# michal-szadkowski/rl-selfplay-mnk

Measured on AMD Instinct MI355X. Metric: env-steps/sec 9x9x5, 65536 parallel envs/GPU, random-policy rollout, higher is better.
Workload: dtype u64

## Files before the change

include/mnk_hip.h:

```cpp
#ifndef MNK_HIP_H
#define MNK_HIP_H

#ifndef __HIPCC_RTC__
#include <stddef.h>
#include <stdint.h>
#endif

#ifdef __cplusplus
extern "C" {
#endif

#define MNK_ABI_VERSION 6

#define MNK_OK 0
#define MNK_EINVAL -1
#define MNK_EGEOM -2
#define MNK_ELAUNCH -3
#define MNK_ECOMM -4

#define MNK_ERR_NONE 0
#define MNK_ERR_ACTION_RANGE 1
#define MNK_ERR_ILLEGAL_MOVE 2
#define MNK_ERR_SYMMETRY 3
#define MNK_ERR_VISITS 4
// ... 252 lines not shown
#define MNK_JIT_REPLAY 1
#define MNK_JIT_ROLLOUT_PAIR 2
int64_t mnk_jit_compile_kernel(int m, int n, int k, int record, int act_bytes, int kind);
const char* mnk_jit_last_error(void);
#define MNK_JIT_API_STEP 0
#define MNK_JIT_API_STEP_DRAW 1
#define MNK_JIT_API_STEP_SUBSET 2
#define MNK_JIT_API_OBSERVE 3
#define MNK_JIT_API_SAMPLE_LEGAL 4
#define MNK_JIT_API_UNPACK_RECORDS 5
#define MNK_JIT_API_GATHER_OBS 6
#define MNK_JIT_API_SP_PRE 7
#define MNK_JIT_API_SP_POST 8
#define MNK_JIT_API_SP_STEP 9
#define MNK_JIT_API_SP_DRAW 10
#define MNK_JIT_API_SP_TACTICAL 19
#define MNK_JIT_API_SP_TACTICAL_DRAW 20
#define MNK_JIT_API_SAMPLE_TACTICAL 23
#define MNK_JIT_API_COUNT 24
int64_t mnk_jit_compile_api(int m, int n, int k, int kind);
int mnk_jit_prepare(int m, int n, int k, int64_t kinds);
int mnk_jit_stats(int64_t* out4);
int mnk_jit_api_ready(int m, int n, int k, int kind);

int mnk_action_log_words(int act_bytes, int T);
int mnk_replay_actions(uint64_t* planes, uint32_t* meta, int64_t N, int m, int n, int k, int T,
                       const void* act_log, int act_bytes, uint64_t* rec_planes, uint32_t* rec_meta,
                       int32_t* err, void* stream);

int mnk_unpack_records(const uint64_t* rec_planes, const uint32_t* rec_meta, int64_t N, int T, int m, int n,
                       void* obs, int obs_dtype, uint8_t* masks, int64_t* actions, float* rewards, uint8_t* dones,
                       void* stream);

int mnk_gather_obs(const uint64_t* planes, int64_t T, int64_t N, int m, int n, const int64_t* idx, int64_t B,
                   void* obs, int obs_dtype, uint8_t* legal_mask, int fix_empty_mask, int32_t* err, void* stream);

int mnk_gae(const float* rewards, const float* values, const uint8_t* dones, const float* last_values,
            int64_t N, int T, float gamma, float gamma_lambda, float* advantages, float* returns,
            void* stream);

int mnk_comm_unique_id(void* id_out_host);
int mnk_comm_init(void** comm_out, const void* id_host, int nranks, int rank);
int mnk_comm_destroy(void* comm);
int mnk_allgather_records(void* comm, const void* send, void* recv, int64_t bytes, void* stream);
int mnk_allgather_records_direct(void* comm, const void* send, void* recv, int64_t bytes, void* stream);
const char* mnk_comm_last_error(void);
int mnk_comm_version(void);

int mnk_probe_record_writes(uint64_t* rec, int64_t N, int T, int rows, void* stream);

int mnk_probe_select_bits(const uint32_t* words, int nw, int64_t count, const int32_t* ranks, int32_t* bits, uint32_t* hot,
                          void* stream);

#ifdef __cplusplus
}
#endif
#endif
```

rl-selfplay-mnk_amd/csrc/mnk_device.h:

```cpp
#pragma once
#ifdef __HIPCC_RTC__
typedef unsigned char uint8_t;
typedef unsigned short uint16_t;
typedef unsigned int uint32_t;
typedef unsigned long long uint64_t;
typedef signed char int8_t;
typedef int int32_t;
typedef long long int64_t;
typedef unsigned long long uintptr_t;
#include "mnk_hip.h"
#else
#include <hip/hip_runtime.h>
#include <stdint.h>

#include "../../include/mnk_hip.h"
#endif

#define MNK_MAX_W 16
#define MNK_MAX_NW 32

struct MnkGeom {
  int m, n, k;
  int C;
  int W;
// ... 123 lines not shown
#pragma unroll
    for (int w = 0; w < NW; ++w) lj[w] = ~0u;
#pragma unroll UK
    for (int j = 0; j < k; ++j) {
      if (j > 0) {
        uint32_t t[NW];
#pragma unroll
        for (int w = 0; w < NW; ++w) t[w] = plane[w];
        bs_shl<NW>(t, j * d);
#pragma unroll
        for (int w = 0; w < NW; ++w) lj[w] &= t[w];
      }
      uint32_t rj[NW];
#pragma unroll
      for (int w = 0; w < NW; ++w) rj[w] = ~0u;
#pragma unroll UK
      for (int i = 1; i < k - j; ++i) {
        uint32_t t[NW];
#pragma unroll
        for (int w = 0; w < NW; ++w) t[w] = plane[w];
        bs_shr<NW>(t, i * d);
#pragma unroll
        for (int w = 0; w < NW; ++w) rj[w] &= t[w];
      }
#pragma unroll
      for (int w = 0; w < NW; ++w) acc[w] |= lj[w] & rj[w];
    }
  }
#pragma unroll
  for (int w = 0; w < NW; ++w) out[w] = acc[w] & empty[w];
}

#define MNK_SELECT_LEVEL(S)                        \
  "v_bfe_u32 %[t], %[x], %[pos], " #S "\n\t"       \
  "v_bcnt_u32_b32 %[t], %[t], %[nr]\n\t"          \
  "v_max_u32 %[nr], %[nr], %[t]\n\t"              \
  "v_ashrrev_i32 %[t], 31, %[t]\n\t"              \
  "v_and_or_b32 %[pos], %[t], " #S ", %[pos]\n\t"
__device__ __forceinline__ uint32_t select_bit32_nr(uint32_t x, uint32_t nr, uint32_t base) {
  uint32_t pos, t;
  asm("v_and_b32 %[t], 0xffff, %[x]\n\t"
      "v_bcnt_u32_b32 %[t], %[t], %[nr]\n\t"
      "v_max_u32 %[nr], %[nr], %[t]\n\t"
      "v_ashrrev_i32 %[t], 31, %[t]\n\t"
      "v_and_or_b32 %[pos], %[t], 16, %[base]\n\t"
      MNK_SELECT_LEVEL(8) MNK_SELECT_LEVEL(4) MNK_SELECT_LEVEL(2)
      "v_bfe_u32 %[t], %[x], %[pos], 1\n\t"
      "v_bitop3_b32 %[t], %[nr], %[t], %[t] bitop3:0x3f\n\t"
      "v_and_or_b32 %[pos], %[t], 1, %[pos]"
      : [pos] "=&v"(pos), [t] "=&v"(t), [nr] "+v"(nr)
      : [x] "v"(x), [base] "v"(base));
  return pos;
}
#undef MNK_SELECT_LEVEL

__device__ __forceinline__ int select_bit32(uint32_t x, int r) { return (int)select_bit32_nr(x, ~(uint32_t)r, 0u); }

template <int NW>
__device__ __forceinline__ int bs_popcount(const uint32_t (&x)[NW]) {
  int c = 0;
#pragma unroll
  for (int w = 0; w < NW; ++w) c += __popc(x[w]);
  return c;
}

template <int NW>
__device__ __forceinline__ int bs_select_hot(const uint32_t (&x)[NW], int r_, uint32_t (&hot)[NW]) {
  const uint32_t nr = ~(uint32_t)r_;
  uint32_t m[NW + 1], word = x[0], base = 0u, rank = nr, pre = 0u;
  m[0] = ~0u;
  m[NW] = 0u;
#pragma unroll
  for (int w = 1; w < NW; ++w) {
    pre += (uint32_t)__popc(x[w - 1]);
    const uint32_t t = pre + nr;
    m[w] = (uint32_t)((int32_t)t >> 31);
    rank = rank > t ? rank : t;
    word = __builtin_amdgcn_bitop3_b32(m[w], x[w], word, 0xca);
    base = __builtin_amdgcn_bitop3_b32(m[w], 32u * w, base, 0xca);
  }
  const uint32_t pos = select_bit32_nr(word, rank, base);
  const uint32_t one = 1u << (pos & 31u);
#pragma unroll
  for (int w = 0; w < NW; ++w) hot[w] = __builtin_amdgcn_bitop3_b32(one, m[w], m[w + 1], 0x40);
  return (int)pos;
}

template <int NW>
__device__ __forceinline__ int bs_select(const uint32_t (&x)[NW], int r) {
  uint32_t hot[NW];
  return bs_select_hot<NW>(x, r, hot);
}

struct Philox4 { uint32_t v[4]; };

__device__ __forceinline__ uint64_t mnk_mul_wide(uint32_t a, uint32_t m) {
  uint64_t product, carry;
  asm("v_mad_u64_u32 %0, %1, %2, %3, 0" : "=v"(product), "=s"(carry) : "v"(a), "s"(m));
  return product;
}
__device__ __forceinline__ uint64_t mnk_mul_wide_vcc(uint32_t a, uint32_t m) {
  uint64_t product;
  asm("v_mad_u64_u32 %0, vcc, %1, %2, 0" : "=v"(product) : "v"(a), "s"(m) : "vcc");
  return product;
}

#define MNK_PHILOX_M0 0xD2511F53u
#define MNK_PHILOX_M1 0xCD9E8D57u

__device__ __forceinline__ uint64_t philox_first_product(uint32_t c0) { return mnk_mul_wide_vcc(c0, MNK_PHILOX_M0); }

__device__ __forceinline__ Philox4 philox4x32_10_from(uint64_t p0_first, uint32_t c1, uint32_t c2, uint32_t c3,
                                                      uint32_t k0, uint32_t k1) {
  uint64_t A[11], B[11];
  uint32_t n0[11], n2[11];
#define MNK_PHILOX_N0(r) \
  n0[r] = __builtin_amdgcn_bitop3_b32((uint32_t)(B[r] >> 32), (r) == 1 ? c1 : (uint32_t)B[(r) - 1], k0 + ((r) - 1) * 0x9E3779B9u, 0x96)
#define MNK_PHILOX_N2(r) \
  n2[r] = __builtin_amdgcn_bitop3_b32((uint32_t)(A[r] >> 32), (r) == 1 ? c3 : (uint32_t)A[(r) - 1], k1 + ((r) - 1) * 0xBB67AE85u, 0x96)
  A[1] = p0_first;
  B[1] = mnk_mul_wide(c2, MNK_PHILOX_M1);
  MNK_PHILOX_N2(1);
#pragma unroll
  for (int r = 2; r <= 10; r += 2) {
    B[r] = mnk_mul_wide(n2[r - 1], MNK_PHILOX_M1);
    MNK_PHILOX_N0(r - 1);
    A[r] = mnk_mul_wide_vcc(n0[r - 1], MNK_PHILOX_M0);
    MNK_PHILOX_N0(r);
    if (r < 10) {
      A[r + 1] = mnk_mul_wide_vcc(n0[r], MNK_PHILOX_M0);
      MNK_PHILOX_N2(r);
      B[r + 1] = mnk_mul_wide(n2[r], MNK_PHILOX_M1);
      MNK_PHILOX_N2(r + 1);
    }
  }
  MNK_PHILOX_N2(10);
#undef MNK_PHILOX_N0
#undef MNK_PHILOX_N2
  Philox4 o;
  o.v[0] = n0[10]; o.v[1] = (uint32_t)B[10]; o.v[2] = n2[10]; o.v[3] = (uint32_t)A[10];
  return o;
}

__device__ __forceinline__ Philox4 philox4x32_10(uint32_t c0, uint32_t c1, uint32_t c2, uint32_t c3,
                                                 uint32_t k0, uint32_t k1) {
#pragma unroll
  for (int r = 0; r < 10; ++r) {
    const uint64_t p0 = mnk_mul_wide(c0, MNK_PHILOX_M0), p1 = mnk_mul_wide(c2, MNK_PHILOX_M1);
    const uint32_t n0 = __builtin_amdgcn_bitop3_b32((uint32_t)(p1 >> 32), c1, k0, 0x96);
    const uint32_t n2 = __builtin_amdgcn_bitop3_b32((uint32_t)(p0 >> 32), c3, k1, 0x96);
    c0 = n0; c1 = (uint32_t)p1; c2 = n2; c3 = (uint32_t)p0;
    k0 += 0x9E3779B9u; k1 += 0xBB67AE85u;
  }
  Philox4 o;
  o.v[0] = c0; o.v[1] = c1; o.v[2] = c2; o.v[3] = c3;
  return o;
}

__device__ __forceinline__ Philox4 mnk_rng_block(uint64_t seed, uint64_t env, uint64_t q, uint32_t stream) {
  return philox4x32_10((uint32_t)env, (uint32_t)(env >> 32), (uint32_t)q,
                       stream | ((uint32_t)((q >> 32) & 0xFFFFFFu) << 8),
                       (uint32_t)seed, (uint32_t)(seed >> 32));
}

__device__ __forceinline__ Philox4 mnk_rng_block_from(uint64_t seed, uint64_t env_p0, uint64_t env, uint64_t q,
                                                      uint32_t stream) {
  return philox4x32_10_from(env_p0, (uint32_t)(env >> 32), (uint32_t)q,
                            stream | ((uint32_t)((q >> 32) & 0xFFFFFFu) << 8),
                            (uint32_t)seed, (uint32_t)(seed >> 32));
}

__device__ __forceinline__ uint32_t philox_word(const Philox4& b, uint32_t i) {
  uint32_t lo = (i & 1u) ? b.v[1] : b.v[0];
  uint32_t hi = (i & 1u) ? b.v[3] : b.v[2];
  return (i & 2u) ? hi : lo;
}

__device__ __forceinline__ uint32_t mnk_rand_u32(uint64_t seed, uint64_t env, uint64_t step, uint32_t stream) {
  Philox4 b = mnk_rng_block(seed, env, step >> 2, stream);
  return philox_word(b, (uint32_t)(step & 3));
}

template <int NW>
struct MnkEnv {
  uint32_t p[2][NW];
  uint32_t meta;
};

template <int NW, bool EXACT = false>
__device__ __forceinline__ void plane_load(uint32_t (&x)[NW], const uint64_t* plane, int64_t N, int W, int64_t i) {
#pragma unroll
  for (int q = 0; q < (NW + 1) / 2; ++q) {
    const uint64_t v = (EXACT || q < W) ? plane[(int64_t)q * N + i] : 0ull;
    x[2 * q] = (uint32_t)v;
    if (2 * q + 1 < NW) x[2 * q + 1] = (uint32_t)(v >> 32);
  }
}

template <int NW, bool EXACT = false>
__device__ __forceinline__ void plane_store(const uint32_t (&x)[NW], uint64_t* plane, int64_t N, int W, int64_t i) {
#pragma unroll
  for (int q = 0; q < (NW + 1) / 2; ++q) {
    const uint64_t hi = (2 * q + 1 < NW) ? (uint64_t)x[2 * q + 1] : 0ull;
    if (EXACT || q < W) plane[(int64_t)q * N + i] = (uint64_t)x[2 * q] | (hi << 32);
  }
}

template <int NW, bool EXACT = false>
__device__ __forceinline__ void rec_store(const uint32_t (&p0)[NW], const uint32_t (&p1)[NW], uint64_t* rows, int64_t N,
                                          int nw, int64_t i) {
#pragma unroll
  for (int w = 0; w < NW; ++w)
    if (EXACT || w < nw) rows[(int64_t)w * N + i] = (uint64_t)p0[w] | ((uint64_t)p1[w] << 32);
}

template <int NW, bool EXACT = false>
__device__ __forceinline__ void rec_load(uint32_t (&p0)[NW], uint32_t (&p1)[NW], const uint64_t* rows, int64_t N, int nw,
                                         int64_t i) {
#pragma unroll
  for (int w = 0; w < NW; ++w) {
    const uint64_t v = (EXACT || w < nw) ? rows[(int64_t)w * N + i] : 0ull;
    p0[w] = (uint32_t)v;
// ... 131 lines not shown
```

rl-selfplay-mnk_amd/csrc/mnk_kernels.hip:

```cpp
#include "mnk_host.h"
#include "mnk_api_kernels.h"
#include "mnk_selfplay_host.h"

__global__ void k_reset_idx(uint64_t* planes, uint32_t* meta, int64_t N, int W, const int64_t* idx, int64_t R,
                            int32_t* err) {
  const int64_t j = (int64_t)blockIdx.x * blockDim.x + threadIdx.x;
  if (j >= R) return;
  int64_t i = idx[j];
  if (i < 0) i += N;
  if (i < 0 || i >= N) { mnk_report(err, MNK_ERR_ACTION_RANGE, idx[j]); return; }
  for (int w = 0; w < 2 * W; ++w) planes[(int64_t)w * N + i] = 0ull;
  meta[i] = 0u;
}

__global__ void k_reset_mask(uint64_t* planes, uint32_t* meta, int64_t N, int W, const uint8_t* mask) {
  const int64_t i = (int64_t)blockIdx.x * blockDim.x + threadIdx.x;
  if (i >= N || !mask[i]) return;
  for (int w = 0; w < 2 * W; ++w) planes[(int64_t)w * N + i] = 0ull;
  meta[i] = 0u;
}

__global__ void k_pack_boards(MnkGeom g, const float* boards, uint64_t* planes, int64_t N) {
  const int64_t i = (int64_t)blockIdx.x * blockDim.x + threadIdx.x;
  if (i >= N) return;
// ... 71 lines not shown
    next_v = v;
  }
}

__global__ void __launch_bounds__(64) k_probe_record_writes(uint64_t* rec, int64_t N, int T, int rows, uint64_t seed) {
  const int64_t i = (int64_t)blockIdx.x * 64 + threadIdx.x;
  if (i >= N) return;
  uint64_t v = seed + (uint64_t)i;
  uint64_t* p = rec + i;
  for (int t = 0; t < T; ++t)
    for (int r = 0; r < rows; ++r) {
      __builtin_nontemporal_store(v + (uint64_t)r, p);
      p += N;
    }
}

template <int NW>
__global__ void __launch_bounds__(64) k_probe_select_bits(const uint32_t* words, int64_t count, const int32_t* ranks,
                                                          int32_t* bits, uint32_t* hot) {
  const int64_t i = (int64_t)blockIdx.x * 64 + threadIdx.x;
  if (i >= count) return;
  uint32_t x[NW], h[NW];
#pragma unroll
  for (int w = 0; w < NW; ++w) x[w] = words[i * NW + w];
  bits[i] = bs_select_hot<NW>(x, ranks[i], h);
#pragma unroll
  for (int w = 0; w < NW; ++w) hot[i * NW + w] = h[w];
}

extern "C" {

int mnk_probe_record_writes(uint64_t* rec, int64_t N, int T, int rows, void* stream) {
  if (!rec || N < 0 || T < 0 || rows < 1) return MNK_EINVAL;
  if (N == 0 || T == 0) return MNK_OK;
  hipLaunchKernelGGL(k_probe_record_writes, dim3((unsigned)((N + 63) / 64)), dim3(64), 0, (hipStream_t)stream, rec, N, T,
                     rows, 0x9E3779B97F4A7C15ull);
  return mnk_launch_status("probe_record_writes");
}

int mnk_probe_select_bits(const uint32_t* words, int nw, int64_t count, const int32_t* ranks, int32_t* bits, uint32_t* hot,
                          void* stream) {
  if (!words || !ranks || !bits || !hot || count < 0 || (nw != 1 && nw != 3 && nw != 12)) return MNK_EINVAL;
  if (count == 0) return MNK_OK;
  const dim3 grid((unsigned)((count + 63) / 64));
  if (nw == 1)
    hipLaunchKernelGGL(k_probe_select_bits<1>, grid, dim3(64), 0, (hipStream_t)stream, words, count, ranks, bits, hot);
  else if (nw == 3)
    hipLaunchKernelGGL(k_probe_select_bits<3>, grid, dim3(64), 0, (hipStream_t)stream, words, count, ranks, bits, hot);
  else
    hipLaunchKernelGGL(k_probe_select_bits<12>, grid, dim3(64), 0, (hipStream_t)stream, words, count, ranks, bits, hot);
  return mnk_launch_status("probe_select_bits");
}

int mnk_abi_version(void) { return MNK_ABI_VERSION; }

int mnk_reload_config(void) {
  mnk_config(true);
  return MNK_OK;
}

int mnk_record_words(int m, int n) {
  MnkGeom g;
  if (mnk_check_geom(m, n, 1, &g) != MNK_OK) return 0;
  return g.NW;
}

int mnk_state_words(int m, int n) {
  if (m < 1 || n < 1 || n > 61) return 0;
  const int W = (m * (n + 1) + 63) / 64;
  return W <= MNK_MAX_W ? W : 0;
}

int mnk_geometry_supported(int m, int n, int k) {
  MnkGeom g;
  return mnk_check_geom(m, n, k, &g) == MNK_OK ? 1 : 0;
}

const char* mnk_last_launch_error(void) { return g_launch_err; }

int mnk_reset_all(uint64_t* planes, uint32_t* meta, int64_t N, int W, void* stream) {
  if (!planes || !meta || N < 0 || W < 1 || W > MNK_MAX_W) return MNK_EINVAL;
  if (N == 0) return MNK_OK;
  hipStream_t s = (hipStream_t)stream;
  if (hipMemsetAsync(planes, 0, (size_t)2 * W * N * sizeof(uint64_t), s) != hipSuccess) return mnk_launch_status("reset_all");
  if (hipMemsetAsync(meta, 0, (size_t)N * sizeof(uint32_t), s) != hipSuccess) return mnk_launch_status("reset_all");
  return MNK_OK;
}

int mnk_reset_idx(uint64_t* planes, uint32_t* meta, int64_t N, int W, const int64_t* idx, int64_t R, int32_t* err,
                  void* stream) {
  if (!planes || !meta || N < 0 || R < 0 || W < 1 || W > MNK_MAX_W || (R > 0 && !idx)) return MNK_EINVAL;
  if (R == 0 || N == 0) return MNK_OK;
  const int B = 256;
  hipLaunchKernelGGL(k_reset_idx, dim3((unsigned)((R + B - 1) / B)), dim3(B), 0, (hipStream_t)stream, planes, meta, N,
                     W, idx, R, err);
  return mnk_launch_status("reset_idx");
}

int mnk_reset_mask(uint64_t* planes, uint32_t* meta, int64_t N, int W, const uint8_t* mask, void* stream) {
  if (!planes || !meta || !mask || N < 0 || W < 1 || W > MNK_MAX_W) return MNK_EINVAL;
  if (N == 0) return MNK_OK;
  const int B = 256;
  hipLaunchKernelGGL(k_reset_mask, dim3((unsigned)((N + B - 1) / B)), dim3(B), 0, (hipStream_t)stream, planes, meta, N,
                     W, mask);
  return mnk_launch_status("reset_mask");
}
// ... 239 lines not shown
```

rl-selfplay-mnk_amd/csrc/mnk_rollout_lane.h:

```cpp
#pragma once
#include "mnk_device.h"
#include "mnk_pair_scan.h"

template <int NW, int CN, int CK, bool RECORD, int ACT = 0, bool PAIR = false, int WS = 1, bool SADDR = false>
struct RolloutLane {
  static constexpr bool EXACT = CN != 0;
  const MnkGeom& g;
  uint32_t cur[NW], oth[NW];
  uint32_t side, moves;
  int64_t N;
  uint32_t role = 0;
  uint32_t wrole = 0;
  uint32_t* vx = nullptr;
  uint64_t* rp = nullptr;
  uint32_t* rm = nullptr;
  static constexpr bool OFF32 = SADDR || PAIR;
  const char* rbase[OFF32 ? NW : 1] = {};
  const char* mbase = nullptr;
  uint32_t roff = 0, moff = 0;
  uint8_t* ra = nullptr;
  uint64_t quad = 0;
  uint32_t q32 = 0;
  uint8_t* rh = nullptr;
  uint32_t hi4 = 0, hiw = 0, hfill = 0;
  uint32_t lo = 0;
  uint32_t fill = 0;
  uint32_t acc_dw = 0, acc_white = 0;
  uint32_t moves_in = 0;
  uint32_t moves_parity = 0;

  __device__ __forceinline__ RolloutLane(const MnkGeom& g_, int64_t N_, int64_t i, uint64_t* rec_planes,
                                         uint32_t* rec_meta, void* act_log, uint32_t role_ = 0, uint32_t wrole_ = 0,
                                         uint32_t* vx_ = nullptr)
      : g(g_), N(N_), role(role_), wrole(wrole_), vx(vx_) {
    if (RECORD) {
      if (!PAIR) rp = rec_planes + i;
      rm = rec_meta + i;
      if (OFF32) {
#pragma unroll
        for (int w = 0; w < NW; ++w) rbase[w] = (const char*)(rec_planes + (int64_t)w * N);
        mbase = (const char*)rec_meta;
        roff = (uint32_t)i * 8u + (PAIR ? role * 4u : 0u);
        moff = (uint32_t)i * 4u;
      }
    }
    static_assert((ACT != 3 && ACT != 4) || (!PAIR && WS == 1), "the bit-packed action logs are built into the one-lane form only");
    if (ACT) ra = (uint8_t*)act_log + i * 4 * (ACT == 2 ? 2 : 1);
  }

  __device__ __forceinline__ void log_begin(void* act_log, int T, int64_t i) {
    if constexpr (ACT == 4) rh = (uint8_t*)act_log + ((int64_t)((T + 3) >> 2) * N + i) * 4;
  }

  __device__ __forceinline__ void load(const uint64_t* planes, const uint32_t* meta, int64_t i) {
    uint32_t p0[NW], p1[NW];
    plane_load<NW, EXACT>(p0, planes, N, g.W, i);
    plane_load<NW, EXACT>(p1, planes + (int64_t)g.W * N, N, g.W, i);
    const uint32_t mw = meta[i];
    side = mw & 1u;
    moves = moves_in = mw >> 1;
#pragma unroll
    for (int w = 0; w < NW; ++w) {
      cur[w] = side ? p1[w] : p0[w];
      oth[w] = side ? p0[w] : p1[w];
    }
  }
// ... 54 lines not shown
    } else {
      store_planes(planes, i);
    }
    meta[i] = (moves << 1) | side;
  }

  __device__ __forceinline__ void log_flush() {
    if constexpr (ACT == 3) {
      if (fill == 0u) {
        lo = q32;
        fill = 28u;
      } else {
        *(uint32_t*)ra = lo | (q32 << fill);
        ra += N * 4;
        lo = q32 >> (32u - fill);
        fill -= 4u;
      }
      q32 = 0;
      return;
    }
    if constexpr (ACT == 4) {
      *(uint32_t*)ra = q32;
      ra += N * 4;
      q32 = 0;
      hiw |= hi4 << hfill;
      hi4 = 0;
      hfill += 4u;
      if (hfill == 32u) {
        *(uint32_t*)rh = hiw;
        rh += N * 4;
        hiw = 0;
        hfill = 0;
      }
      return;
    }
    if (WS == 1 || wrole == 0) {
      if (ACT == 1) *(uint32_t*)ra = (uint32_t)quad;
      if (ACT == 2) *(uint64_t*)ra = quad;
    }
    ra += N * 4 * ACT;
    quad = 0;
  }

  __device__ __forceinline__ void log_finish(int T) {
    if (ACT && (T & 3)) log_flush();
    if constexpr (ACT == 3) {
      if (fill) *(uint32_t*)ra = lo;
    }
    if constexpr (ACT == 4) {
      if (hfill) *(uint32_t*)rh = hiw;
    }
  }

  template <bool FAST = false>
  __device__ __forceinline__ int pick(uint32_t x, uint32_t (&hot)[NW], uint32_t& nlegal) const {
    uint32_t legal[NW];
#pragma unroll
    for (int w = 0; w < NW; ++w) legal[w] = ~(cur[w] | oth[w]) & g.valid[w];
    const int nl = bs_popcount<NW>(legal);
    nlegal = (uint32_t)nl;
    int n = nl;
    if (!FAST && __builtin_amdgcn_ballot_w64(nl == 0) != 0) {
#pragma unroll
      for (int w = 0; w < NW; ++w) legal[w] = nl ? legal[w] : g.valid[w];
      n = nl ? nl : g.C;
    }
    const int r = (int)__umulhi(x, (uint32_t)n);
    const uint32_t bit = (uint32_t)bs_select_hot<NW>(legal, r, hot);
    return mnk_bit_cell<CN>(g, bit);
  }

  template <bool FAST = false>
  __device__ __forceinline__ void ply(uint32_t x, int field) {
    uint32_t hot[NW];
    uint32_t nlegal;
    const int a = pick<FAST>(x, hot, nlegal);
    if constexpr (ACT == 3) {
      q32 |= (uint32_t)a << (7 * field);
      if (field == 3) log_flush();
    } else if constexpr (ACT == 4) {
      q32 |= ((uint32_t)a & 0xFFu) << (8 * field);
      hi4 |= ((uint32_t)a >> 8) << field;
      if (field == 3) log_flush();
    } else if (ACT) {
      quad |= (uint64_t)(uint32_t)a << (8 * ACT * field);
      if (field == 3) log_flush();
    }
    ply_hot<FAST>(a, hot, nlegal);
  }

  __device__ __forceinline__ void ply_action(int a) {
    ply_bit(a, mnk_cell_bit<CN>(g, (uint32_t)a));
  }

  __device__ __forceinline__ void ply_bit(int a, uint32_t bit) {
    const int wsel = (int)(bit >> 5);
    const uint32_t one = 1u << (bit & 31u);
    uint32_t hot[NW];
#pragma unroll
    for (int w = 0; w < NW; ++w) hot[w] = (w == wsel) ? one : 0u;
    ply_hot<false>(a, hot);
  }

  template <bool FAST = false>
  __device__ __forceinline__ void ply_hot(int a, const uint32_t (&hot)[NW], uint32_t nlegal = 0) {
    if (RECORD) store_record();
#pragma unroll
    for (int w = 0; w < NW; ++w) cur[w] |= hot[w];
    if (!FAST) ++moves;
    uint32_t win;
    if constexpr (PAIR) {
      uint32_t hit = bs_run_bits_pair<NW, CK, CN + 1, CN + 2>(cur, role) | bs_run_bits_pair<NW, CK, 1, CN>(cur, role);
      hit |= pair_swap(hit);
      win = hit ? 1u : 0u;
    } else if constexpr (WS > 1) {
      bool hit = false;
      if constexpr (WS == 4) {
        if (wrole == 0) hit = bs_has_run<NW>(cur, 1, CK);
        else if (wrole == 1) hit = bs_has_run<NW>(cur, CN + 1, CK);
        else if (wrole == 2) hit = bs_has_run<NW>(cur, CN + 2, CK);
        else hit = bs_has_run<NW>(cur, CN, CK);
      } else {
        if (wrole == 0) hit = bs_has_run<NW>(cur, 1, CK) | bs_has_run<NW>(cur, CN + 1, CK);
        else hit = bs_has_run<NW>(cur, CN + 2, CK) | bs_has_run<NW>(cur, CN, CK);
      }
      uint32_t* slot = vx + ((moves_parity & 1u) * 64u + (threadIdx.x & 63u)) * WS;
      slot[wrole] = hit ? 1u : 0u;
      asm volatile("s_waitcnt lgkmcnt(0)\n\ts_barrier" ::: "memory");
      uint32_t any = 0;
#pragma unroll
      for (int r = 0; r < WS; ++r) any |= slot[r];
      win = any;
      ++moves_parity;
    } else {
      win = mnk_plane_wins<NW, CN, CK>(g, cur) ? 1u : 0u;
    }
    const uint32_t done = win | ((FAST ? nlegal == 1u : moves >= (uint32_t)g.C) ? 1u : 0u);
    const uint32_t mover = FAST ? (((uint32_t)g.C ^ nlegal) & 1u) : side;
    if (RECORD) {
      const uint32_t mword = (uint32_t)a | (win << MNK_REC_REWARD_SHIFT) | (done << MNK_REC_DONE_BIT) | (mover << MNK_REC_SIDE_BIT);
      if constexpr (OFF32) {
        __builtin_nontemporal_store(mword, (uint32_t*)(mbase + (uint64_t)moff));
        moff += (uint32_t)N * 4u;
      } else {
        if (WS == 1 || wrole == WS - 1) __builtin_nontemporal_store(mword, rm);
        rm += N;
      }
    }
    acc_dw += done | (win << 16);
    static_assert(MNK_REC_REWARD_SHIFT == 16, "the FAST white-win count multiplies the meta word's win bit, taken to be bit 16");
    if (FAST) asm("v_mad_u32_u24 %0, %1, %2, %0" : "+v"(acc_white) : "v"(win << 16), "v"(mover));
    else acc_white += win & side;
#pragma unroll
    for (int w = 0; w < NW; ++w) {
      const uint32_t c = cur[w];
      cur[w] = done ? 0u : oth[w];
      oth[w] = done ? 0u : c;
    }
    if (!FAST) {
      side = done ? 0u : (side ^ 1u);
      moves = done ? 0u : moves;
    }
  }

  __device__ __forceinline__ uint32_t acc_done() const { return acc_dw & 0xFFFFu; }
  __device__ __forceinline__ uint32_t acc_win() const { return acc_dw >> 16; }

  __device__ __forceinline__ bool consistent() const {
    uint32_t occ[NW];
#pragma unroll
    for (int w = 0; w < NW; ++w) occ[w] = cur[w] | oth[w];
    return (uint32_t)bs_popcount<NW>(occ) == moves && moves < (uint32_t)g.C && side == (moves & 1u);
  }

  __device__ __forceinline__ void finish_fast() {
    uint32_t occ[NW];
#pragma unroll
    for (int w = 0; w < NW; ++w) occ[w] = cur[w] | oth[w];
    moves = (uint32_t)bs_popcount<NW>(occ);
    side = moves & 1u;
    acc_white >>= 16;
  }
};

template <bool FAST, bool LEAN = FAST, typename Lane>
__device__ __forceinline__ void rollout_plies(Lane& L, int T, uint64_t seed, uint64_t step0, uint64_t env) {
  int t = 0;
  uint64_t step = step0;
  uint64_t env_p0 = 0;
  if constexpr (LEAN) env_p0 = philox_first_product((uint32_t)env);
  auto block = [&](uint64_t q) {
    if constexpr (LEAN) return mnk_rng_block_from(seed, env_p0, env, q, MNK_STREAM_MOVE);
    else return mnk_rng_block(seed, env, q, MNK_STREAM_MOVE);
  };
  if (step & 3) {
    const Philox4 blk = block(step >> 2);
    for (; t < T && (step & 3); ++t, ++step)
      L.template ply<FAST>(philox_word(blk, (uint32_t)(step & 3)), (int)(step & 3));
  }
  if constexpr (FAST) {
    const int blocks = (T - t) >> 2;
    uint64_t q = step >> 2;
    for (int left = blocks; left > 0; --left, ++q) {
      const Philox4 blk = block(q);
      L.template ply<FAST>(blk.v[0], 0);
      L.template ply<FAST>(blk.v[1], 1);
      L.template ply<FAST>(blk.v[2], 2);
      L.template ply<FAST>(blk.v[3], 3);
    }
    t += blocks << 2;
    step += (uint64_t)blocks << 2;
  } else {
    for (; t + 4 <= T; t += 4, step += 4) {
      const Philox4 blk = block(step >> 2);
      L.template ply<FAST>(blk.v[0], 0);
      L.template ply<FAST>(blk.v[1], 1);
      L.template ply<FAST>(blk.v[2], 2);
      L.template ply<FAST>(blk.v[3], 3);
    }
  }
  if (t < T) {
    const Philox4 blk = block(step >> 2);
    for (uint32_t j = 0; t < T; ++t, ++j) L.template ply<FAST>(philox_word(blk, j), (int)j);
  }
}

template <int NW, int CN, int CK, bool RECORD, int ACT, bool SADDR = false>
__device__ __forceinline__ void rollout_random_body(const MnkGeom& g, uint64_t* planes, uint32_t* meta, int64_t N, int T,
                                                    uint64_t seed, uint64_t step0, int64_t env_id0,
                                                    uint64_t* rec_planes, uint32_t* rec_meta, unsigned long long* stats,
                                                    void* act_log) {
  __shared__ unsigned int lds_stats[MNK_STATS_COUNTERS];
  if (threadIdx.x < MNK_STATS_COUNTERS) lds_stats[threadIdx.x] = 0u;
  __syncthreads();
  const int64_t i = (int64_t)blockIdx.x * blockDim.x + threadIdx.x;
  if (i < N) {
    RolloutLane<NW, CN, CK, RECORD, ACT, false, 1, SADDR> L(g, N, i, rec_planes, rec_meta, act_log);
    L.log_begin(act_log, T, i);
    L.load(planes, meta, i);
    const uint64_t env = (uint64_t)(env_id0 + i);
    constexpr bool TRY_FAST = NW <= 3 || (NW == 6 && CN == 13);
    if (TRY_FAST && __builtin_amdgcn_ballot_w64(!L.consistent()) == 0) {
      rollout_plies<true>(L, T, seed, step0, env);
      L.finish_fast();
    } else {
      rollout_plies<false, TRY_FAST>(L, T, seed, step0, env);
    }
    L.log_finish(T);
    L.store(planes, meta, i);
    if (stats) {
      const uint32_t len_sum = L.moves_in + (uint32_t)T - L.moves;
      if (L.acc_done()) atomicAdd(&lds_stats[0], L.acc_done());
      if (L.acc_win() - L.acc_white) atomicAdd(&lds_stats[1], L.acc_win() - L.acc_white);
      if (L.acc_white) atomicAdd(&lds_stats[2], L.acc_white);
      if (L.acc_done() - L.acc_win()) atomicAdd(&lds_stats[3], L.acc_done() - L.acc_win());
      if (len_sum) atomicAdd(&lds_stats[4], len_sum);
    }
  }
  __syncthreads();
  if (stats && threadIdx.x < MNK_STATS_COUNTERS && lds_stats[threadIdx.x])
    atomicAdd(&stats[(size_t)(blockIdx.x % MNK_STATS_REPLICAS) * MNK_STATS_STRIDE + threadIdx.x],
              (unsigned long long)lds_stats[threadIdx.x]);
}

template <bool FAST, bool LEAN = FAST, typename Lane>
__device__ __forceinline__ void pair_plies(Lane& L, int T, uint64_t seed, uint64_t step0, uint64_t env, uint32_t role) {
  int t = 0;
  uint64_t step = step0;
  uint64_t env_p0 = 0;
  if constexpr (LEAN) env_p0 = philox_first_product((uint32_t)env);
  for (; t < T && (step & 7); ++t, ++step)
    L.template ply<FAST>(mnk_rand_u32(seed, env, step, MNK_STREAM_MOVE), (int)(step & 3));
  for (; t + 8 <= T; t += 8, step += 8) {
    const Philox4 mine = LEAN ? mnk_rng_block_from(seed, env_p0, env, (step >> 2) + role, MNK_STREAM_MOVE)
                              : mnk_rng_block(seed, env, (step >> 2) + role, MNK_STREAM_MOVE);
    uint32_t lo[4], hi[4];
#pragma unroll
    for (int j = 0; j < 4; ++j) {
      const uint32_t other = pair_swap(mine.v[j]);
      lo[j] = role ? other : mine.v[j];
      hi[j] = role ? mine.v[j] : other;
    }
#pragma unroll
    for (int j = 0; j < 4; ++j) L.template ply<FAST>(lo[j], j);
#pragma unroll
    for (int j = 0; j < 4; ++j) L.template ply<FAST>(hi[j], j);
  }
  for (; t < T; ++t, ++step) L.template ply<FAST>(mnk_rand_u32(seed, env, step, MNK_STREAM_MOVE), (int)(step & 3));
}

// ... 175 lines not shown
```

rl-selfplay-mnk_amd/mnk_hip/__init__.py:

```python
import ctypes
import os

import torch

_HERE = os.path.dirname(os.path.abspath(__file__))
LIB_PATH = os.environ.get("MNK_HIP_LIB") or os.path.join(_HERE, "libmnk_hip.so")
ABI_VERSION = 6

MNK_OK = 0
ERR_NONE, ERR_ACTION_RANGE, ERR_ILLEGAL_MOVE, ERR_SYMMETRY, ERR_VISITS = 0, 1, 2, 3, 4
STEP_STRICT, STEP_AUTORESET = 1, 2
LOGITS_F32, LOGITS_BF16 = 0, 1
OBS_F32, OBS_BF16, OBS_U8 = 0, 1, 2
ACT_U8, ACT_U16, ACT_BITS7, ACT_U8P1 = 1, 2, 3, 4
COMM_ID_BYTES = 128
SP_NEED_OPP, SP_WAS_RESET = 1, 2
STREAM_MOVE, STREAM_OPP, STREAM_SIDE, STREAM_SAMPLE, STREAM_PLAYOUT, STREAM_SEARCH, STREAM_SELFPLAY = 0, 1, 2, 3, 4, 5, 6
STREAM_NOISE = 7
Z_UNKNOWN = -128
PROOF_UNKNOWN = -128
PLAYOUTS_MAX = 4096
SEARCH_ITERS_MAX = 2048
SEARCH_PLAYOUTS_MAX = 256
PUCT_ITERS_MAX = 2048
# ... 56 lines not shown
    "mnk_puct_workspace_bytes": [_i64, _i, _i, _i],
    "mnk_puct_begin": [_vp, _i, _i64, _i, _i, _i, _i, _vp, _vp, _i, _vp, _vp],
    "mnk_puct_rebase": [_vp, _i, _i64, _i, _i, _i, _i, _i, _vp, _vp, _i, _vp, _vp, _vp],
    "mnk_puct_step": [_vp, _i64, _i, _i, _i, _i, _vp, _i, _vp, _i, _f, _i, _i, _u64, _vp, _u64, _vp, _i64, _i, _vp, _i,
                      _vp, _vp, _vp, _vp, _vp],
    "mnk_puct_workspace_bytes_leaves": [_i64, _i, _i, _i, _i],
    "mnk_puct_begin_leaves": [_vp, _i, _i64, _i, _i, _i, _i, _i, _vp, _vp, _i, _vp, _vp],
    "mnk_puct_rebase_leaves": [_vp, _i, _i64, _i, _i, _i, _i, _i, _i, _vp, _vp, _i, _vp, _vp, _vp],
    "mnk_puct_step_leaves": [_vp, _i64, _i, _i, _i, _i, _i, _vp, _i, _vp, _i, _f, _i, _i, _u64, _vp, _u64, _vp, _i64, _i,
                             _vp, _i, _vp, _vp, _vp, _vp, _vp],
    "mnk_puct_step_solver": [_vp, _i64, _i, _i, _i, _i, _i, _vp, _i, _vp, _i, _f, _i, _i, _u64, _vp, _u64, _vp, _i64, _i,
                             _vp, _i, _vp, _vp, _vp, _vp, _vp, _vp],
    "mnk_puct_root_noise": [_vp, _i, _vp, _i64, _i, _i, _f, _f, _u64, _vp, _u64, _vp, _i64, _vp, _vp],
    "mnk_puct_gumbel_schedule": [_i, _i, _vp],
    "mnk_puct_gumbel_root": [_vp, _i, _vp, _vp, _i, _i64, _i, _f, _u64, _vp, _u64, _vp, _i64, _vp, _vp, _vp],
    "mnk_puct_step_gumbel": [_vp, _i64, _i, _i, _i, _i, _i, _vp, _i, _vp, _i, _f, _i, _i, _f, _f, _vp, _vp, _vp, _u64, _vp,
                             _u64, _vp, _i64, _i, _vp, _i, _vp, _vp, _vp, _vp, _vp, _vp],
    "mnk_search_selfplay_step_moves": [_vp, _vp, _i64, _i, _i, _i, _vp, _vp, _u64, _vp, _i64, _vp, _vp, _vp, _vp, _i, _vp,
                                       _vp, _vp, _vp],
    "mnk_search_selfplay_step": [_vp, _vp, _i64, _i, _i, _i, _vp, _i, _u64, _vp, _u64, _vp, _i64, _i64, _vp, _vp, _vp, _vp,
                                 _i, _vp, _vp, _vp, _vp],
    "mnk_search_selfplay_advance": [_vp, _vp, _vp, _i64, _i, _i, _i, _i, _i, _u64, _vp, _i, _vp, _i, _f, _i, _u64, _vp, _i64,
                                    _vp, _i64, _vp, _vp, _vp, _vp, _i, _vp, _vp, _vp, _vp, _vp, _vp],
    "mnk_search_selfplay_advance_opts": [_vp, _vp, _vp, _i64, _i, _i, _i, _i, _i, _u64, _vp, _i, _vp, _i, _f, _i, _u64, _vp,
                                         _i64, _vp, _i64, _vp, _vp, _vp, _vp, _i, _vp, _vp, _vp, _vp, _vp, _i, _f, _f, _i,
                                         _vp, _vp],
    "mnk_search_selfplay_advance_keep": [_vp, _vp, _vp, _i64, _i, _i, _i, _i, _i, _u64, _vp, _i, _vp, _i, _f, _i, _u64, _vp,
                                         _i64, _vp, _i64, _vp, _vp, _vp, _vp, _i, _vp, _vp, _vp, _vp, _vp, _i, _f, _f, _i,
                                         _vp, _i, _i, _vp, _vp],
    "mnk_search_gather": [_vp, _vp, _vp, _i64, _i64, _i, _i, _vp, _vp, _i64, _vp, _i, _vp, _vp, _vp, _vp, _vp, _vp],
    "mnk_rollout_random": [_vp, _vp, _i64, _i, _i, _i, _i, _u64, _u64, _i64, _vp, _vp, _vp, _vp, _i, _vp],
    "mnk_rollout_form": [_i64, _i, _i, _i, _i, _i, _i, _i],
    "mnk_action_log_words": [_i, _i],
    "mnk_replay_actions": [_vp, _vp, _i64, _i, _i, _i, _i, _vp, _i, _vp, _vp, _vp, _vp],
    "mnk_unpack_records": [_vp, _vp, _i64, _i, _i, _i, _vp, _i, _vp, _vp, _vp, _vp, _vp],
    "mnk_gather_obs": [_vp, _i64, _i64, _i, _i, _vp, _i64, _vp, _i, _vp, _i, _vp, _vp],
    "mnk_gae": [_vp, _vp, _vp, _vp, _i64, _i, _f, _f, _vp, _vp, _vp],
    "mnk_jit_compile_rollout": [_i, _i, _i, _i, _i],
    "mnk_jit_compile_kernel": [_i, _i, _i, _i, _i, _i],
    "mnk_jit_last_error": [],
    "mnk_jit_compile_api": [_i, _i, _i, _i],
    "mnk_jit_prepare": [_i, _i, _i, _i64],
    "mnk_jit_api_ready": [_i, _i, _i, _i],
    "mnk_jit_stats": [_vp],
    "mnk_comm_unique_id": [_vp],
    "mnk_comm_init": [_vp, _vp, _i, _i],
    "mnk_comm_destroy": [_vp],
    "mnk_allgather_records": [_vp, _vp, _vp, _i64, _vp],
    "mnk_allgather_records_direct": [_vp, _vp, _vp, _i64, _vp],
    "mnk_comm_last_error": [],
    "mnk_comm_version": [],
    "mnk_probe_record_writes": [_vp, _i64, _i, _i, _vp],
    "mnk_probe_select_bits": [_vp, _i, _i64, _vp, _vp, _vp, _vp],
}

_STATUS = {-1: "invalid argument (null pointer / negative size)", -2: "unsupported board geometry",
           -3: "kernel launch failed", -4: "RCCL call failed"}


class MnkHipError(RuntimeError):
    pass


_lib = None


def load():
    global _lib
    if _lib is not None:
        return _lib
    if not os.path.exists(LIB_PATH):
        raise MnkHipError(
            f"{LIB_PATH} is missing: build it with `python -c 'import __graft_entry__ as g; g.build()'` "
            "(hipcc --offload-arch=gfx950).  There is no CPU fallback for this path."
        )
    lib = ctypes.CDLL(LIB_PATH)
    for name, argtypes in SIGNATURES.items():
        try:
            fn = getattr(lib, name)
        except AttributeError:
            if os.environ.get("MNK_HIP_LIB"):
                continue
            raise
        fn.argtypes = argtypes
        if name in ("mnk_last_launch_error", "mnk_comm_last_error", "mnk_jit_last_error"):
            fn.restype = ctypes.c_char_p
        elif name in ("mnk_jit_compile_rollout", "mnk_jit_compile_kernel", "mnk_jit_compile_api",
                      "mnk_puct_workspace_bytes", "mnk_puct_workspace_bytes_leaves"):
            fn.restype = ctypes.c_int64
        else:
            fn.restype = ctypes.c_int
    if lib.mnk_abi_version() != ABI_VERSION:
        raise MnkHipError(f"libmnk_hip.so ABI {lib.mnk_abi_version()} != binding ABI {ABI_VERSION}")
    _lib = lib
    return lib


def ptr(t):
    if t is None:
        return None
    assert t.is_contiguous(), "mnk_hip: tensors handed to the C ABI must be contiguous"
    return t.data_ptr()


_raw_stream = getattr(torch._C, "_cuda_getCurrentRawStream", None)

# ... 111 lines not shown
```

Baseline: 208.8 billion.

## Use LDS byte-select table and interleave next Philox block into select latency

Replaces the last three levels of the in-register bit-select with a 2 KB LDS lookup table of bit positions per byte, filled once per workgroup, for boards with at most 3 words. The LDS load latency is covered by running slices of the next Philox block's statements, plus the record store, between scheduling barriers. This software-pipelines RNG generation across the four plies of a block. It adds LDS use and register pressure from keeping the next Philox state live, and the fill assumes a block of at least 64 threads.

```diff
diff --git a/include/mnk_hip.h b/include/mnk_hip.h
--- a/include/mnk_hip.h
+++ b/include/mnk_hip.h
@@ -328,6 +328,8 @@
 int mnk_probe_select_bits(const uint32_t* words, int nw, int64_t count, const int32_t* ranks, int32_t* bits, uint32_t* hot,
                           void* stream);
 
+int mnk_probe_select_table(uint8_t* out);
+
 #ifdef __cplusplus
 }
 #endif
diff --git a/rl-selfplay-mnk_amd/csrc/mnk_device.h b/rl-selfplay-mnk_amd/csrc/mnk_device.h
--- a/rl-selfplay-mnk_amd/csrc/mnk_device.h
+++ b/rl-selfplay-mnk_amd/csrc/mnk_device.h
@@ -199,6 +199,50 @@
       : [x] "v"(x), [base] "v"(base));
   return pos;
 }
+struct MnkSelectTable {
+  uint8_t t[256][8];
+  constexpr MnkSelectTable() : t() {
+    for (int b = 0; b < 256; ++b) {
+      int r = 0;
+      for (int p = 0; p < 8; ++p)
+        if ((b >> p) & 1) t[b][r++] = (uint8_t)p;
+    }
+  }
+};
+#define MNK_SELECT_TABLE_BYTES 2048
+static __device__ const MnkSelectTable mnk_select_table_rom = MnkSelectTable();
+
+__device__ __forceinline__ void mnk_select_table_fill(uint32_t* lds_table) {
+  const uint4* src = (const uint4*)&mnk_select_table_rom.t[0][0];
+  uint4* dst = (uint4*)lds_table;
+  dst[threadIdx.x] = src[threadIdx.x];
+  dst[threadIdx.x + 64u] = src[threadIdx.x + 64u];
+}
+
+struct MnkNoCover {
+  __device__ __forceinline__ void operator()() const {}
+};
+template <typename Cover>
+__device__ __forceinline__ uint32_t select_bit32_nr_tab(uint32_t x, uint32_t nr, uint32_t base, const uint8_t* tab,
+                                                        Cover&& cover) {
+  uint32_t pos, t;
+  asm("v_and_b32 %[t], 0xffff, %[x]\n\t"
+      "v_bcnt_u32_b32 %[t], %[t], %[nr]\n\t"
+      "v_max_u32 %[nr], %[nr], %[t]\n\t"
+      "v_ashrrev_i32 %[t], 31, %[t]\n\t"
+      "v_and_or_b32 %[pos], %[t], 16, %[base]\n\t"
+      MNK_SELECT_LEVEL(8)
+      "v_bfe_u32 %[t], %[x], %[pos], 8\n\t"
+      "v_not_b32 %[nr], %[nr]\n\t"
+      "v_lshl_add_u32 %[t], %[t], 3, %[nr]"
+      : [pos] "=&v"(pos), [t] "=&v"(t), [nr] "+v"(nr)
+      : [x] "v"(x), [base] "v"(base));
+  const uint32_t in_byte = tab[t];
+  __builtin_amdgcn_sched_barrier(0);
+  cover();
+  __builtin_amdgcn_sched_barrier(0);
+  return pos | in_byte;
+}
 #undef MNK_SELECT_LEVEL
 
 __device__ __forceinline__ int select_bit32(uint32_t x, int r) { return (int)select_bit32_nr(x, ~(uint32_t)r, 0u); }
@@ -211,8 +255,9 @@
   return c;
 }
 
-template <int NW>
-__device__ __forceinline__ int bs_select_hot(const uint32_t (&x)[NW], int r_, uint32_t (&hot)[NW]) {
+template <int NW, bool TAB = false, typename Cover = MnkNoCover>
+__device__ __forceinline__ int bs_select_hot(const uint32_t (&x)[NW], int r_, uint32_t (&hot)[NW],
+                                             const uint8_t* tab = nullptr, Cover&& cover = Cover()) {
   const uint32_t nr = ~(uint32_t)r_;
   uint32_t m[NW + 1], word = x[0], base = 0u, rank = nr, pre = 0u;
   m[0] = ~0u;
@@ -226,7 +271,9 @@
     word = __builtin_amdgcn_bitop3_b32(m[w], x[w], word, 0xca);
     base = __builtin_amdgcn_bitop3_b32(m[w], 32u * w, base, 0xca);
   }
-  const uint32_t pos = select_bit32_nr(word, rank, base);
+  uint32_t pos;
+  if constexpr (TAB) pos = select_bit32_nr_tab(word, rank, base, tab, cover);
+  else pos = select_bit32_nr(word, rank, base);
   const uint32_t one = 1u << (pos & 31u);
 #pragma unroll
   for (int w = 0; w < NW; ++w) hot[w] = __builtin_amdgcn_bitop3_b32(one, m[w], m[w + 1], 0x40);
@@ -256,6 +303,52 @@
 #define MNK_PHILOX_M1 0xCD9E8D57u
 
 __device__ __forceinline__ uint64_t philox_first_product(uint32_t c0) { return mnk_mul_wide_vcc(c0, MNK_PHILOX_M0); }
+
+struct PhiloxSteps {
+  static constexpr int COUNT = 39;
+  uint64_t A[11], B[11];
+  uint32_t n0[11], n2[11];
+  uint32_t c1, c2, c3, k0, k1;
+  __device__ __forceinline__ PhiloxSteps(uint64_t p0_first, uint32_t c1_, uint32_t c2_, uint32_t c3_, uint32_t k0_,
+                                         uint32_t k1_)
+      : c1(c1_), c2(c2_), c3(c3_), k0(k0_), k1(k1_) {
+    A[1] = p0_first;
+  }
+  __device__ __forceinline__ void xor_n0(int r) {
+    n0[r] = __builtin_amdgcn_bitop3_b32((uint32_t)(B[r] >> 32), r == 1 ? c1 : (uint32_t)B[r - 1],
+                                        k0 + (uint32_t)(r - 1) * 0x9E3779B9u, 0x96);
+  }
+  __device__ __forceinline__ void xor_n2(int r) {
+    n2[r] = __builtin_amdgcn_bitop3_b32((uint32_t)(A[r] >> 32), r == 1 ? c3 : (uint32_t)A[r - 1],
+                                        k1 + (uint32_t)(r - 1) * 0xBB67AE85u, 0x96);
+  }
+  __device__ __forceinline__ void statement(int s) {
+    if (s == 0) { B[1] = mnk_mul_wide(c2, MNK_PHILOX_M1); return; }
+    if (s == 1) { xor_n2(1); return; }
+    if (s == 38) { xor_n2(10); return; }
+    const int r = 2 + 2 * ((s - 2) >> 3);
+    switch ((s - 2) & 7) {
+      case 0: B[r] = mnk_mul_wide(n2[r - 1], MNK_PHILOX_M1); break;
+      case 1: xor_n0(r - 1); break;
+      case 2: A[r] = mnk_mul_wide_vcc(n0[r - 1], MNK_PHILOX_M0); break;
+      case 3: xor_n0(r); break;
+      case 4: A[r + 1] = mnk_mul_wide_vcc(n0[r], MNK_PHILOX_M0); break;
+      case 5: xor_n2(r); break;
+      case 6: B[r + 1] = mnk_mul_wide(n2[r], MNK_PHILOX_M1); break;
+      default: xor_n2(r + 1); break;
+    }
+  }
+  template <int FROM, int TO>
+  __device__ __forceinline__ void run() {
+#pragma unroll
+    for (int s = FROM; s < TO; ++s) statement(s);
+  }
+  __device__ __forceinline__ Philox4 words() const {
+    Philox4 o;
+    o.v[0] = n0[10]; o.v[1] = (uint32_t)B[10]; o.v[2] = n2[10]; o.v[3] = (uint32_t)A[10];
+    return o;
+  }
+};
 
 __device__ __forceinline__ Philox4 philox4x32_10_from(uint64_t p0_first, uint32_t c1, uint32_t c2, uint32_t c3,
                                                       uint32_t k0, uint32_t k1) {
@@ -315,6 +408,12 @@
   return philox4x32_10_from(env_p0, (uint32_t)(env >> 32), (uint32_t)q,
                             stream | ((uint32_t)((q >> 32) & 0xFFFFFFu) << 8),
                             (uint32_t)seed, (uint32_t)(seed >> 32));
+}
+
+__device__ __forceinline__ PhiloxSteps mnk_rng_steps_from(uint64_t seed, uint64_t env_p0, uint64_t env, uint64_t q,
+                                                          uint32_t stream) {
+  return PhiloxSteps(env_p0, (uint32_t)(env >> 32), (uint32_t)q, stream | ((uint32_t)((q >> 32) & 0xFFFFFFu) << 8),
+                     (uint32_t)seed, (uint32_t)(seed >> 32));
 }
 
 __device__ __forceinline__ uint32_t philox_word(const Philox4& b, uint32_t i) {
diff --git a/rl-selfplay-mnk_amd/csrc/mnk_kernels.hip b/rl-selfplay-mnk_amd/csrc/mnk_kernels.hip
--- a/rl-selfplay-mnk_amd/csrc/mnk_kernels.hip
+++ b/rl-selfplay-mnk_amd/csrc/mnk_kernels.hip
@@ -147,6 +147,14 @@
   return mnk_launch_status("probe_select_bits");
 }
 
+int mnk_probe_select_table(uint8_t* out) {
+  if (!out) return MNK_EINVAL;
+  static constexpr MnkSelectTable table = MnkSelectTable();
+  static_assert(sizeof(table.t) == MNK_SELECT_TABLE_BYTES, "the LDS copy is filled 2 KB at a time");
+  memcpy(out, &table.t[0][0], sizeof(table.t));
+  return MNK_OK;
+}
+
 int mnk_abi_version(void) { return MNK_ABI_VERSION; }
 
 int mnk_reload_config(void) {
diff --git a/rl-selfplay-mnk_amd/csrc/mnk_rollout_lane.h b/rl-selfplay-mnk_amd/csrc/mnk_rollout_lane.h
--- a/rl-selfplay-mnk_amd/csrc/mnk_rollout_lane.h
+++ b/rl-selfplay-mnk_amd/csrc/mnk_rollout_lane.h
@@ -2,9 +2,11 @@
 #include "mnk_device.h"
 #include "mnk_pair_scan.h"
 
-template <int NW, int CN, int CK, bool RECORD, int ACT = 0, bool PAIR = false, int WS = 1, bool SADDR = false>
+template <int NW, int CN, int CK, bool RECORD, int ACT = 0, bool PAIR = false, int WS = 1, bool SADDR = false,
+          bool SELTAB = false>
 struct RolloutLane {
   static constexpr bool EXACT = CN != 0;
+  static constexpr bool TABLE = SELTAB;
   const MnkGeom& g;
   uint32_t cur[NW], oth[NW];
   uint32_t side, moves;
@@ -12,6 +14,7 @@
   uint32_t role = 0;
   uint32_t wrole = 0;
   uint32_t* vx = nullptr;
+  const uint8_t* seltab = nullptr;
   uint64_t* rp = nullptr;
   uint32_t* rm = nullptr;
   static constexpr bool OFF32 = SADDR || PAIR;
@@ -172,8 +175,8 @@
     }
   }
 
-  template <bool FAST = false>
-  __device__ __forceinline__ int pick(uint32_t x, uint32_t (&hot)[NW], uint32_t& nlegal) const {
+  template <bool FAST = false, typename Cover = MnkNoCover>
+  __device__ __forceinline__ int pick(uint32_t x, uint32_t (&hot)[NW], uint32_t& nlegal, Cover&& cover = Cover()) const {
     uint32_t legal[NW];
 #pragma unroll
     for (int w = 0; w < NW; ++w) legal[w] = ~(cur[w] | oth[w]) & g.valid[w];
@@ -186,15 +189,18 @@
       n = nl ? nl : g.C;
     }
     const int r = (int)__umulhi(x, (uint32_t)n);
-    const uint32_t bit = (uint32_t)bs_select_hot<NW>(legal, r, hot);
+    const uint32_t bit = (uint32_t)bs_select_hot<NW, SELTAB>(legal, r, hot, seltab, cover);
     return mnk_bit_cell<CN>(g, bit);
   }
 
-  template <bool FAST = false>
-  __device__ __forceinline__ void ply(uint32_t x, int field) {
+  template <bool FAST = false, typename Ahead = MnkNoCover>
+  __device__ __forceinline__ void ply(uint32_t x, int field, Ahead&& ahead = Ahead()) {
     uint32_t hot[NW];
     uint32_t nlegal;
-    const int a = pick<FAST>(x, hot, nlegal);
+    const int a = pick<FAST>(x, hot, nlegal, [&]() {
+      ahead();
+      if (RECORD) store_record();
+    });
     if constexpr (ACT == 3) {
       q32 |= (uint32_t)a << (7 * field);
       if (field == 3) log_flush();
@@ -206,7 +212,7 @@
       quad |= (uint64_t)(uint32_t)a << (8 * ACT * field);
       if (field == 3) log_flush();
     }
-    ply_hot<FAST>(a, hot, nlegal);
+    ply_hot<FAST, SELTAB>(a, hot, nlegal);
   }
 
   __device__ __forceinline__ void ply_action(int a) {
@@ -222,9 +228,9 @@
     ply_hot<false>(a, hot);
   }
 
-  template <bool FAST = false>
+  template <bool FAST = false, bool STORED = false>
   __device__ __forceinline__ void ply_hot(int a, const uint32_t (&hot)[NW], uint32_t nlegal = 0) {
-    if (RECORD) store_record();
+    if (RECORD && !STORED) store_record();
 #pragma unroll
     for (int w = 0; w < NW; ++w) cur[w] |= hot[w];
     if (!FAST) ++moves;
@@ -321,12 +327,24 @@
   if constexpr (FAST) {
     const int blocks = (T - t) >> 2;
     uint64_t q = step >> 2;
-    for (int left = blocks; left > 0; --left, ++q) {
-      const Philox4 blk = block(q);
-      L.template ply<FAST>(blk.v[0], 0);
-      L.template ply<FAST>(blk.v[1], 1);
-      L.template ply<FAST>(blk.v[2], 2);
-      L.template ply<FAST>(blk.v[3], 3);
+    if constexpr (Lane::TABLE && LEAN) {
+      Philox4 blk = block(q);
+      for (int left = blocks; left > 0; --left) {
+        PhiloxSteps next = mnk_rng_steps_from(seed, env_p0, env, ++q, MNK_STREAM_MOVE);
+        L.template ply<FAST>(blk.v[0], 0, [&]() { next.template run<0, 10>(); });
+        L.template ply<FAST>(blk.v[1], 1, [&]() { next.template run<10, 20>(); });
+        L.template ply<FAST>(blk.v[2], 2, [&]() { next.template run<20, 30>(); });
+        L.template ply<FAST>(blk.v[3], 3, [&]() { next.template run<30, PhiloxSteps::COUNT>(); });
+        blk = next.words();
+      }
+    } else {
+      for (int left = blocks; left > 0; --left, ++q) {
+        const Philox4 blk = block(q);
+        L.template ply<FAST>(blk.v[0], 0);
+        L.template ply<FAST>(blk.v[1], 1);
+        L.template ply<FAST>(blk.v[2], 2);
+        L.template ply<FAST>(blk.v[3], 3);
+      }
     }
     t += blocks << 2;
     step += (uint64_t)blocks << 2;
@@ -352,10 +370,18 @@
                                                     void* act_log) {
   __shared__ unsigned int lds_stats[MNK_STATS_COUNTERS];
   if (threadIdx.x < MNK_STATS_COUNTERS) lds_stats[threadIdx.x] = 0u;
+  constexpr bool SELTAB = NW <= 3;
+  const uint8_t* seltab = nullptr;
+  if constexpr (SELTAB) {
+    __shared__ uint32_t lds_seltab[MNK_SELECT_TABLE_BYTES / 4];
+    mnk_select_table_fill(lds_seltab);
+    seltab = (const uint8_t*)lds_seltab;
+  }
   __syncthreads();
   const int64_t i = (int64_t)blockIdx.x * blockDim.x + threadIdx.x;
   if (i < N) {
-    RolloutLane<NW, CN, CK, RECORD, ACT, false, 1, SADDR> L(g, N, i, rec_planes, rec_meta, act_log);
+    RolloutLane<NW, CN, CK, RECORD, ACT, false, 1, SADDR, SELTAB> L(g, N, i, rec_planes, rec_meta, act_log);
+    L.seltab = seltab;
     L.log_begin(act_log, T, i);
     L.load(planes, meta, i);
     const uint64_t env = (uint64_t)(env_id0 + i);
diff --git a/rl-selfplay-mnk_amd/mnk_hip/__init__.py b/rl-selfplay-mnk_amd/mnk_hip/__init__.py
--- a/rl-selfplay-mnk_amd/mnk_hip/__init__.py
+++ b/rl-selfplay-mnk_amd/mnk_hip/__init__.py
@@ -132,6 +132,7 @@
     "mnk_comm_version": [],
     "mnk_probe_record_writes": [_vp, _i64, _i, _i, _vp],
     "mnk_probe_select_bits": [_vp, _i, _i64, _vp, _vp, _vp, _vp],
+    "mnk_probe_select_table": [_vp],
 }
 
 _STATUS = {-1: "invalid argument (null pointer / negative size)", -2: "unsupported board geometry",
```

New measurement: 215.5 billion, median of 6. 3.2% higher.
